# ml-jku/LRAM

Hardware: AMD Instinct MI355X
Metric: env-steps/sec (action-inference) (higher is better)
Workload: dtype f32

## Files before the change

lram_amd/csrc/common.h:

```cpp
#pragma once
#include <hip/hip_runtime.h>
#include <stdint.h>

#include <stdexcept>
#include <string>
#include <type_traits>

namespace lram {

inline bool first_use_on_device(uint64_t& mask) {
  int dev = 0;
  (void)hipGetDevice(&dev);
  const uint64_t bit = 1ull << (dev & 63);
  if (mask & bit) return false;
  mask |= bit;
  return true;
}

struct Error : std::runtime_error {
  using std::runtime_error::runtime_error;
};

#define LRAM_HIP_CHECK(expr)                                                                         \
  do {                                                                                               \
// ... 19 lines not shown
  const float* residual = nullptr;
  int64_t lda = 0, ldw = 0, ldc = 0;
  int m = 0, n = 0, k = 0;
  int nb1 = 1, nb2 = 1;
  int64_t sA1 = 0, sA2 = 0, sW1 = 0, sW2 = 0, sC1 = 0, sC2 = 0, sBias1 = 0, sBias2 = 0;
  const uint16_t* w3 = nullptr;
  int64_t w3_plane = 0;
  const float* gate = nullptr;
  int64_t ldg = 0;
  int act_silu_from = -1;
  const uint16_t* w2 = nullptr;
  int64_t w2_plane = 0, w2_kt = 0;
  const float* w_inv = nullptr;
  const float* a_amax = nullptr;
  int amax_parts = 1;
  const uint16_t* a2 = nullptr;
  int64_t a2_plane = 0, a2_kt = 0;
  const float* a2_inv = nullptr;
  float* splitk_ws = nullptr;
  int64_t splitk_ws_elems = 0;
  const float* a_tab[4] = {nullptr, nullptr, nullptr, nullptr};
  const float* w_tab[4] = {nullptr, nullptr, nullptr, nullptr};
  float* c_tab[4] = {nullptr, nullptr, nullptr, nullptr};
  const uint16_t* w3_tab[4] = {nullptr, nullptr, nullptr, nullptr};
  const float* norm_g = nullptr;
  const float* norm_b = nullptr;
  float norm_eps = 0.f;
  int norm_rms = 0;
  int xcd_gm = 0, xcd_gn = 0;
  int panel_w = 0;
// ... 441 lines not shown
```

lram_amd/csrc/engine.h:

```cpp
#pragma once
#include <algorithm>
#include <array>
#include <cstdlib>
#include <cstring>
#include <map>
#include <memory>
#include <string>
#include <vector>

#include "../../include/lram_hip.h"
#include "common.h"

namespace lram::host {

struct DevBuf {
  float* p = nullptr;
  size_t n = 0;
  void alloc(size_t numel) {
    release();
    if (numel == 0) return;
    LRAM_HIP_CHECK(hipMalloc(reinterpret_cast<void**>(&p), numel * sizeof(float)));
    n = numel;
  }
  void zero(hipStream_t s = nullptr) {
// ... 108 lines not shown
  uint8_t* slot_dev = nullptr;
  int32_t* slot_img_list = nullptr;
  int slot_n_image = 0;
  bool slot_has_discrete = false;
  int lazy_mode = 2;
  bool lazy = false;
  bool lazy_ready = false;
  int lazy_period = 13;
  int gn_fuse = 2;
  bool mamba_dt_fuse = true;
  int slstm_fused_rows = 512;
  int gemm_skinny_rows = 384;
  static constexpr int slstm_gates_rows = 768;
  int gemm_skinny_min = 5;
  static constexpr int gemm_skinny_k = 1024;
  static constexpr int fold_bubbles = 2;
  bool fold_tail = true;
  static constexpr int fold_tail_blocks = 2;
  struct Prefold {
    bool pending = false;
    int blocks = 0;
    int64_t step = 0;
    int period = 0, B = 0;
  } prefold;
  int64_t lazy_step = 0;
  std::vector<int> lazy_bound;
  bool lazy_dirty = false;
  DevBuf LZ_COUNT;
  std::vector<SlotSeg> slot_segs;
  SlotSeg* slot_segs_dev = nullptr;
  SlotChunk* slot_chunks_dev = nullptr;
  int slot_n_chunks = 0, slot_n_rec_chunks = 0;
  int32_t* slot_idx_dev = nullptr;
// ... 168 lines not shown
struct Slice {
  int b0, nb;
  hipStream_t s;
};

struct Pass {
  const uint8_t* images = nullptr;
  int img_c = 0, img_h = 0, img_w = 0;
  bool slots = false;
  int compat_pass = 0, compat_passes = 1;
  bool compat_shared = false;
  const std::vector<hipEvent_t>* lane_wait = nullptr;
  const std::vector<hipEvent_t>* lane_rec = nullptr;
  int n_slices = 1;
  const uint8_t* hold = nullptr;
};

struct ScoreSink {
  float* actions = nullptr;
  int32_t* tokens = nullptr;
  float* logp = nullptr;
  float* logits = nullptr;
  const float* target_actions = nullptr;
  const int32_t* target_tokens = nullptr;
  const uint8_t* valid = nullptr;
  int over = 0;
  double temperature = 1.0;
};

extern thread_local std::string g_last_error;

void alloc_workspace(lram_engine* e, int tokens);
void swap_workspace(lram_engine* e, int lane);
bool twin_ready(lram_engine* e);
int prefill_chunk_steps(lram_engine* e, int L);
bool takes_skinny(const lram_engine* e, const GemmArgs& g);
bool takes_skinny_with_norm(const lram_engine* e, const GemmArgs& g);
bool f16x2_rows(const lram_engine* e, int rows, int n, int k);
bool f16x2_weight(const lram_engine* e, const float* w, int ldw, GemmArgs* g);
bool presplit_for(const lram_engine* e, const float* w, int rows, int n, int k);
void gemm(lram_engine* e, GemmArgs& g, hipStream_t s);
void make_split(lram_engine* e, const float* w, size_t n);
hipEvent_t new_event(const lram_engine* e, bool boundary);
void prof_record(lram_engine* e, hipStream_t s, bool start, bool aux = false);
void prof_tick(lram_engine* e);
hipEvent_t ring_event(lram_engine* e, bool boundary = false);
void stream_after(lram_engine* e, hipStream_t dst, hipStream_t src, bool boundary = false);
std::vector<Slice> make_slices(lram_engine* e, hipStream_t s, hipStream_t* hbm);
void fork_slices(lram_engine* e, const std::vector<Slice>& sl, hipStream_t hbm, hipStream_t s);
void join_slices(lram_engine* e, const std::vector<Slice>& sl, hipStream_t hbm, hipStream_t s);
void save_slot_records(lram_engine* e, const int32_t* host_slots, int n, float* dev_records, hipStream_t s);
void load_slot_records(lram_engine* e, const int32_t* host_slots, int n, const float* dev_records, hipStream_t s);
void lazy_materialize(lram_engine* e, hipStream_t s);
void lazy_finish_prefold(lram_engine* e, hipStream_t s);
void run_xlstm_stack(lram_engine* e, const Pass& pass, int T, const uint8_t* reset, const std::vector<Slice>& sl, hipStream_t hbm);
void run_mamba_stack(lram_engine* e, const Pass& pass, int T, const uint8_t* reset, const std::vector<Slice>& sl);

inline bool has_mlstm_block(const lram_engine* e) {
  if (e->cfg.backbone != LRAM_BACKBONE_XLSTM) return false;
  for (int i = 0; i < e->cfg.n_blocks; ++i)
    if (!e->cfg.block_is_slstm[i]) return true;
  return false;
}
inline double mlstm_block_bytes(const lram_engine* e) {
  if (!has_mlstm_block(e)) return 0.0;
  const double dh = (double)e->cfg.inner / e->cfg.n_heads;
  return (double)e->B * e->cfg.n_heads * dh * dh * 4.0;
}

inline double mlstm_live_bytes(const lram_engine* e) {
  if (!has_mlstm_block(e)) return 0.0;
// ... 36 lines not shown
```

lram_amd/csrc/engine.hip:

```cpp
#include "engine.h"

namespace {

const float* need(lram_engine* e, const std::string& name, size_t numel) {
  auto it = e->weights.find(name);
  if (it == e->weights.end()) throw Error("lram: missing weight '" + name + "'");
  if (it->second.n != numel)
    throw Error("lram: weight '" + name + "' has " + std::to_string(it->second.n) + " elements, expected " +
                std::to_string(numel));
  return it->second.p;
}
const float* optional(lram_engine* e, const std::string& name, size_t numel) {
  auto it = e->weights.find(name);
  if (it == e->weights.end()) return nullptr;
  if (it->second.n != numel)
    throw Error("lram: weight '" + name + "' has " + std::to_string(it->second.n) + " elements, expected " +
                std::to_string(numel));
  return it->second.p;
}

void validate_config(const lram_config& c) {
  LRAM_REQUIRE(c.abi_version == LRAM_ABI_VERSION, "config.abi_version does not match the library");
  LRAM_REQUIRE(c.backbone == LRAM_BACKBONE_XLSTM || c.backbone == LRAM_BACKBONE_MAMBA, "unknown backbone");
  LRAM_REQUIRE(c.d_model > 0 && c.d_model % 4 == 0 && c.d_model <= 2048, "d_model must be a multiple of 4, <= 2048");
// ... 451 lines not shown
  return mlstm_block_bytes(e) >= 128.0 * 1024 * 1024;
}

struct Knob {
  const char* name;
  void (*set)(lram_engine& e, const char* v);
};
const Knob kKnobs[] = {
    {"LRAM_STATE", [](lram_engine& e, const char* v) {
       const std::string m(v);
       e.lazy_mode = m == "lazy" ? 1 : (m == "eager" || m == "materialised" || m == "materialized") ? 0 : 2;
     }},
    {"LRAM_LAZY_PERIOD", [](lram_engine& e, const char* v) { e.lazy_period = std::max(1, std::min(14, std::atoi(v))); }},
    {"LRAM_LAZY_CAP2_ENVS", [](lram_engine& e, const char* v) { e.lazy_cap2_envs = std::max(0, std::atoi(v)); }},
    {"LRAM_FOLD_TAIL", [](lram_engine& e, const char* v) { e.fold_tail = std::atoi(v) != 0; }},
    {"LRAM_GN_FUSE", [](lram_engine& e, const char* v) { e.gn_fuse = std::max(0, std::min(2, std::atoi(v))); }},
    {"LRAM_F16_MIN_ROWS", [](lram_engine& e, const char* v) { e.f16x2_min_rows = std::max(9, std::atoi(v)); }},
    {"LRAM_GEMM_PRESPLIT", [](lram_engine& e, const char* v) { e.gemm_presplit = std::atoi(v) != 0; }},
    {"LRAM_GEMM_NARROW", [](lram_engine& e, const char* v) { e.gemm_narrow_on = std::atoi(v) != 0, e.gemm_narrow_f16 = std::atoi(v) != 2; }},
    {"LRAM_UPZ_8P", [](lram_engine& e, const char* v) { e.upz_beside = std::atoi(v) != 0; }},
    {"LRAM_SLSTM_GATES_ONE", [](lram_engine& e, const char* v) { e.slstm_gates_one = std::atoi(v) != 0; }},
    {"LRAM_GN_AMAX", [](lram_engine& e, const char* v) { e.gn_amax_handover = std::atoi(v) != 0, e.gn_planes = std::atoi(v) >= 2; }},
    {"LRAM_GEMM_SKINNY_ROWS", [](lram_engine& e, const char* v) { e.gemm_skinny_rows = std::max(0, std::atoi(v)); }},
    {"LRAM_GEMM_SKINNY_MIN", [](lram_engine& e, const char* v) { e.gemm_skinny_min = std::max(1, std::atoi(v)); }},
    {"LRAM_SLSTM_FUSED_ROWS", [](lram_engine& e, const char* v) { e.slstm_fused_rows = std::max(0, std::atoi(v)); }},
    {"LRAM_SLSTM_SEQ", [](lram_engine& e, const char* v) { e.slstm_seq = std::atoi(v) != 0, e.slstm_seq_f32 = std::atoi(v) == 2; }},
    {"LRAM_FRONT_MULTI", [](lram_engine& e, const char* v) { e.front_multi = std::atoi(v) != 0; }},
    {"LRAM_FRONT_MIN_ENVS", [](lram_engine& e, const char* v) { e.front_min_envs = std::max(1, std::atoi(v)); }},
    {"LRAM_MAMBA_DT_FUSE", [](lram_engine& e, const char* v) { e.mamba_dt_fuse = std::atoi(v) != 0; }},
    {"LRAM_COMPAT_SHARE", [](lram_engine& e, const char* v) { e.compat_share = std::atoi(v) != 0; }},
// ... 25 lines not shown
      s.conv.alloc((size_t)B * c.conv_k * D);
    } else {
      const size_t DH = e->dh();
      s.s0.alloc((size_t)B * c.n_heads * DH * DH);
      s.n.alloc((size_t)B * c.inner);
      s.m.alloc((size_t)B * c.n_heads);
      s.conv.alloc((size_t)B * c.conv_k * c.inner);
    }
    s.s0.zero();
    s.n.zero();
    s.m.zero();
    s.conv.zero();
  }
  e->B = B;
  e->n_live = B;
  alloc_workspace(e, kMaxTokens);
  e->lazy = lazy_choice(e);
  if (e->lazy) lazy_alloc(e);
  if (e->slot_segs_dev == nullptr) slot_segments_build(e);
  LRAM_HIP_CHECK(hipDeviceSynchronize());
}

}

extern "C" {

const char* lram_last_error(void) { return g_last_error.c_str(); }

int32_t lram_abi_version(void) { return LRAM_ABI_VERSION; }

// ... 251 lines not shown
```

lram_amd/csrc/engine_gemm.hip:

```cpp
#include "engine.h"

namespace lram::host {

bool takes_skinny(const lram_engine* e, const GemmArgs& g) {
  const bool shape = g.k <= e->gemm_skinny_k && (g.m <= e->gemm_skinny_rows / 2 || (int64_t)g.n * g.k <= 600000);
  return g.m >= e->gemm_skinny_min && g.m <= e->gemm_skinny_rows && shape && gemm_skinny_supported(g);
}
bool takes_skinny_with_norm(const lram_engine* e, const GemmArgs& g) {
  return takes_skinny(e, g) && gemm_skinny_norm_supported(g);
}

}

namespace {

bool narrow_takes(const lram_engine* e, const GemmArgs& g) {
  if (!e->gemm_narrow_on || g.m < e->gemm_narrow_min_rows || g.a2 != nullptr || (int)g.ldw != g.k) return false;
  return e->narrow.count(g.w) != 0 && gemm_narrow_supported(g);
}

}

namespace lram::host {

// ... 11 lines not shown
  if (g != nullptr) {
    g->w2 = it->second.planes + row0 * 32;
    g->w2_plane = (int64_t)split_f16x2_plane_elems(it->second.rows, it->second.k), g->w2_kt = (int64_t)it->second.rows * 32;
    g->w_inv = it->second.inv + row0;
  }
  return true;
}

bool presplit_for(const lram_engine* e, const float* w, int rows, int n, int k) {
  if (!e->gemm_presplit || (k & 31) != 0 || e->XN2.p == nullptr || !f16x2_rows(e, rows, n, k)) return false;
  GemmArgs probe;
  if ((int64_t)e->XN2.n * 4 >= (1ll << 31) || !f16x2_weight(e, w, k, &probe)) return false;
  return 4 * probe.w2_plane < (1ll << 31);
}

void gemm(lram_engine* e, GemmArgs& g, hipStream_t s) {
  if (e->SK.p != nullptr) {
    g.splitk_ws = e->SK.p + (size_t)stream_slot(e, s) * lram_engine::kSplitKSlotElems;
    g.splitk_ws_elems = (int64_t)lram_engine::kSplitKSlotElems;
  }
  if (g.a2 != nullptr) {
    LRAM_REQUIRE(f16x2_weight(e, g.w, (int)g.ldw, &g) && gemm_f16x2p_supported(g),
                 "gemm: pre-split A operand for a projection the pre-split kernel does not serve");
    launch_gemm_f16x2p(g, s);
    count_gemm(e, 0, g);
    return;
  }
  if (narrow_takes(e, g)) {
    if (e->use_f16x2 && e->gemm_narrow_f16 && g.a_amax != nullptr && f16x2_weight(e, g.w, (int)g.ldw, &g) && gemm_narrow16_supported(g)) {
      launch_gemm_narrow16(g, s);
      count_gemm(e, 0, g);
      return;
    }
    g.w2 = nullptr, g.w_inv = nullptr, g.w2_kt = 0;
    launch_gemm_narrow(g, e->narrow.find(g.w)->second.p, s);
    count_gemm(e, 2, g);
    return;
  }
  if (f16x2_rows(e, g.m, g.n, g.k) && g.nb1 * g.nb2 == 1 && e->ASCALE.p != nullptr && (size_t)g.m <= e->ascale_rows) {
    if (f16x2_weight(e, g.w, (int)g.ldw, &g) && gemm_f16x2_supported(g)) {
      if (g.a_amax == nullptr) {
        float* sc = e->ASCALE.p + (size_t)stream_slot(e, s) * e->ascale_rows;
        launch_row_amax(g.a, g.lda, g.gate, g.ldg, g.m, g.k, sc, s);
        g.a_amax = sc, g.amax_parts = 1;
      }
      launch_gemm_f16x2(g, s);
      count_gemm(e, 0, g);
      return;
    }
    g.w2 = nullptr, g.w_inv = nullptr, g.w2_kt = 0;
  }
  if (takes_skinny(e, g)) {
    launch_gemm_skinny(g, s);
    count_gemm(e, 3, g);
    return;
  }
  if (e->use_bf16x3 && !gemm_small_m(g)) {
    auto it = e->split.upper_bound(g.w);
    if (it != e->split.begin() && (--it, g.w < it->first + it->second.n)) {
      g.w3 = it->second.p + (g.w - it->first);
      g.w3_plane = (int64_t)it->second.n;
      if (gemm_bf16x3_supported(g)) {
        launch_gemm_bf16x3(g, s);
        count_gemm(e, 1, g);
        return;
      }
// ... 169 lines not shown
```

lram_amd/csrc/engine_step.hip:

```cpp
#include "engine.h"

namespace {

void run_stack(lram_engine* e, Pass pass, int T, const uint8_t* reset, const std::vector<Slice>& sl, hipStream_t hbm) {
  pass.n_slices = (int)sl.size();
  if (e->cfg.backbone == LRAM_BACKBONE_MAMBA)
    run_mamba_stack(e, pass, T, reset, sl);
  else
    run_xlstm_stack(e, pass, T, reset, sl, hbm);
}

struct ImageFrameFloats {
  size_t p, x;
};
ImageFrameFloats image_frame_floats(int H, int W) {
  const size_t hp = (H - 1) / 2 + 1, wp = (W - 1) / 2 + 1;
  const size_t x = 32 * hp * wp;
  return {std::max((size_t)16 * H * W, x), x};
}

void image_buffers(lram_engine* e, int C, int H, int W, const char* who) {
  const std::string wh(who);
  LRAM_REQUIRE(e->img_lin_w != nullptr, wh + ": no embed_image.* weights were uploaded");
  LRAM_REQUIRE(C == e->img_channels, wh + ": channel count " + std::to_string(C) +
// ... 178 lines not shown
  const lram_config& c = e->cfg;
  const int D = c.d_model, T = c.tokens_per_step;
  const int64_t nlog = (int64_t)c.act_dim * c.n_vocab;
  const int pred = T * (last_steps - 1) + c.pred_token;
  const int col_begin = pass.compat_pass;
  const int col_end = (pass.compat_shared && col_begin + 1 < pass.compat_passes) ? col_begin + 1 : c.act_dim;
  const int col0 = pass.compat_shared ? col_begin : 0;
  e->last_head = discrete;
  const HeadGeom geom = head_geom(c);
  for (const Slice& x : sl) {
    const size_t r0 = (size_t)x.b0 * Tc, b0 = x.b0;
    GemmArgs gh;
    gh.a = e->HID.p + (r0 + pred) * D, gh.lda = (int64_t)Tc * D, gh.w = e->w_head + (size_t)col0 * c.n_vocab * D, gh.ldw = D;
    gh.c = e->LOGITS.p + b0 * nlog + (size_t)col0 * c.n_vocab, gh.ldc = nlog, gh.bias = e->b_head + (size_t)col0 * c.n_vocab;
    gh.m = x.nb, gh.n = (col_end - col0) * c.n_vocab, gh.k = D;
    gemm(e, gh, x.s);
    if (sink != nullptr) {
      ScoreArgs a = score_args(e, *sink, discrete);
      a.logits = e->LOGITS.p + b0 * nlog, a.ld = nlog, a.row0 = (int64_t)b0, a.rows = x.nb;
      a.inner = 1, a.outer = L, a.off = L - 1, a.start = ctx_start;
      launch_action_score(a, x.s);
      continue;
    }
    const float* logits = e->LOGITS.p + b0 * nlog;
    float* act = actions + b0 * c.act_dim;
    int32_t* tok = tokens ? tokens + b0 * c.act_dim : nullptr;
    const HeadSlots slots = head_slots(e, discrete, b0);
    if (e->sampling) {
      SampleArgs sp = e->sample;
      sp.slot0 += b0, sp.draw = e->sample_draw;
// ... 132 lines not shown
bool compat_shares(const lram_engine* e, int discrete) {
  const int passes = discrete ? 1 : std::max(1, std::min(e->compat_repeat, e->cfg.act_dim));
  return passes > 1 && e->cfg.backbone == LRAM_BACKBONE_MAMBA && e->compat_share && e->cfg.n_blocks >= 2;
}
void compat_prepare(lram_engine* e, int discrete) {
  if (e->B <= 0 || !compat_shares(e, discrete)) return;
  const size_t bt = (size_t)e->B * e->cfg.tokens_per_step;
  if (e->X0.n < bt * e->cfg.d_model) e->X0.alloc(bt * e->cfg.d_model);
  if (e->U0.n < bt * 2 * e->cfg.d_inner) e->U0.alloc(bt * 2 * e->cfg.d_inner);
}

void step_launches(lram_engine* e, Pass pass, const Inputs& in, const uint8_t* reset, int discrete, float* actions,
                   int32_t* tokens, hipStream_t s) {
  pass.compat_passes = discrete ? 1 : std::max(1, std::min(e->compat_repeat, e->cfg.act_dim));
  pass.compat_shared = compat_shares(e, discrete);
  if (pass.compat_shared) {
    const size_t bt = (size_t)e->n_live * e->cfg.tokens_per_step;
    LRAM_REQUIRE(e->X0.n >= bt * e->cfg.d_model && e->U0.n >= bt * 2 * e->cfg.d_inner,
                 "shared repeated forwards: workspace not prepared");
  }
  for (pass.compat_pass = 0; pass.compat_pass < pass.compat_passes; ++pass.compat_pass)
    timesteps_launches(e, pass, in, pass.compat_pass == 0 ? reset : nullptr, discrete, actions, tokens, s);
  sample_draw_advance(e, s);
}

void require_all_live(const lram_engine* e, const char* who) {
  LRAM_REQUIRE(e->n_live == e->B, std::string(who) + ": " + std::to_string(e->B - e->n_live) + " of " + std::to_string(e->B) +
                                      " env slots are parked (lram_set_live): stored contexts and encoder calls need every slot "
                                      "live -- call lram_set_live(batch) first");
}
// ... 188 lines not shown
        if (!e->capture_stream) LRAM_HIP_CHECK(hipStreamCreateWithFlags(&e->capture_stream, hipStreamNonBlocking));
        hipStream_t cs = e->capture_stream;
        LRAM_HIP_CHECK(hipStreamBeginCapture(cs, hipStreamCaptureModeThreadLocal));
        try {
          step_launches(e, Pass{}, in, dev_reset_mask, discrete, dev_actions, dev_tokens, cs);
        } catch (...) {
          hipGraph_t g = nullptr;
          (void)hipStreamEndCapture(cs, &g);
          if (g) (void)hipGraphDestroy(g);
          throw;
        }
        LRAM_HIP_CHECK(hipStreamEndCapture(cs, &e->graph));
        LRAM_HIP_CHECK(hipGraphInstantiate(&e->graph_exec, e->graph, nullptr, nullptr, 0));
        e->graph_key = key;
        e->graph_valid = true;
      }
      LRAM_HIP_CHECK(hipGraphLaunch(e->graph_exec, s));
    } else {
      step_launches(e, Pass{}, in, dev_reset_mask, discrete, dev_actions, dev_tokens, s);
    }
  });
}

int32_t lram_step_images(lram_engine* e, const uint8_t* dev_images, int32_t channels, int32_t height, int32_t width,
                         const float* dev_rtg, const float* dev_reward, const uint8_t* dev_reset_mask, int32_t discrete,
                         float* dev_actions, int32_t* dev_tokens, void* stream) {
  return guarded([&] {
    step_entry(e, "lram_step_images");
    LRAM_REQUIRE(dev_images && dev_rtg && dev_reward && dev_actions && channels > 0 && height > 0 && width > 0,
                 "lram_step_images: bad argument");
    LRAM_REQUIRE(e->img_lin_w != nullptr, "lram_step_images: no embed_image.* weights were uploaded");
    check_head_mode(e, discrete, "lram_step_images");
// ... 218 lines not shown
    LRAM_HIP_CHECK(hipMemcpyAsync(dev_hidden_out, e->HID.p, bytes, hipMemcpyDeviceToDevice, s));
  });
}

int32_t lram_get_taps(lram_engine* e, float* dev_tokens_embed, float* dev_hidden, float* dev_logits, void* stream) {
  return guarded([&] {
    LRAM_REQUIRE(e && e->B > 0, "lram_get_taps: state not allocated");
    hipStream_t s = static_cast<hipStream_t>(stream);
    const size_t btd = sizeof(float) * (size_t)e->n_live * e->cfg.tokens_per_step * e->cfg.d_model;
    if (dev_tokens_embed) {
      LRAM_REQUIRE(e->B <= kTokenTapMaxBatch,
                   "lram_get_taps: the embed_ln token tap is kept for batches of up to 1024 env slots only (it costs a "
                   "copy of the token buffer per step); pass NULL for it");
      LRAM_HIP_CHECK(hipMemcpyAsync(dev_tokens_embed, e->TOK.p, btd, hipMemcpyDeviceToDevice, s));
    }
    if (dev_hidden) LRAM_HIP_CHECK(hipMemcpyAsync(dev_hidden, e->HID.p, btd, hipMemcpyDeviceToDevice, s));
    if (dev_logits)
      LRAM_HIP_CHECK(hipMemcpyAsync(dev_logits, e->LOGITS.p, sizeof(float) * (e->LOGITS.n / e->B) * e->n_live, hipMemcpyDeviceToDevice, s));
  });
}

int32_t lram_sample_tokens(const float* dev_logits, int64_t rows, int32_t n, int64_t ld, double temperature, int32_t top_k,
                           double top_p, const double* dev_uniform, int32_t* dev_tokens, void* stream) {
  return guarded([&] {
    LRAM_REQUIRE(dev_logits && dev_uniform && dev_tokens, "lram_sample_tokens: null device pointer");
    LRAM_REQUIRE(temperature > 0.0 && temperature < (double)INFINITY, "lram_sample_tokens: temperature must be finite and > 0");
    LRAM_REQUIRE(top_p >= 0.0 && top_p <= 1.0, "lram_sample_tokens: top_p must be in [0, 1]");
    LRAM_REQUIRE(top_k >= 0 && top_k <= n, "lram_sample_tokens: top_k must be in 0 .. n");
    LRAM_REQUIRE(ld == 0 || ld >= n, "lram_sample_tokens: ld must be 0 (one shared row) or >= n");
    launch_sample_tokens(dev_logits, rows, n, ld, temperature, top_k, top_p, dev_uniform, dev_tokens,
                         static_cast<hipStream_t>(stream));
// ... 24 lines not shown
```

lram_amd/csrc/engine_xlstm.hip:

```cpp
#include "engine.h"

namespace {

MlstmLazyArgs lazy_args(lram_engine* e, int i, int T, const uint8_t* reset, int b0, int nb, int step_off = 0) {
  const lram_config& c = e->cfg;
  const size_t NH = c.n_heads, DH = e->dh(), B = e->B;
  const int64_t step = e->lazy_step + step_off;
  const int in = (int)(step & 1), out = 1 - in;
  BlockState& st = e->st[i];
  MlstmLazyArgs a{};
  a.C = st.s0.p + (size_t)b0 * NH * DH * DH;
  a.wk = st.wk.p + (size_t)b0 * NH * kLazyWindow * DH;
  a.wv = st.wv.p + (size_t)b0 * NH * kLazyWindow * DH;
  a.coef_in = st.coef.p + (in * B + b0) * NH * kLazyWindow;
  a.coef_out = st.coef.p + (out * B + b0) * NH * kLazyWindow;
  a.g_in = st.gsc.p + (in * B + b0) * NH;
  a.g_out = st.gsc.p + (out * B + b0) * NH;
  a.count_in = reinterpret_cast<const int32_t*>(e->LZ_COUNT.p) + in * B + b0;
  a.count_out = reinterpret_cast<int32_t*>(e->LZ_COUNT.p) + out * B + b0;
  a.pw = st.pw.p ? st.pw.p + (size_t)b0 * NH * T * kLazyWT : nullptr;
  a.reset = reset ? reset + b0 : nullptr;
  a.B = nb, a.T = T, a.NH = (int)NH, a.DH = (int)DH;
  a.phase = (int)((step + b0) % e->lazy_period), a.period = e->lazy_period, a.force = 0;
  return a;
// ... 174 lines not shown
  ca.reset = reset ? reset + b0 : nullptr, ca.B = sl.nb, ca.T = T, ca.NH = NH, ca.DH = DH;
  ca.hold = pass.hold ? pass.hold + b0 : nullptr;
  const long wgs = (long)sl.nb * NH * ((DH % 256 == 0) ? DH / 256 : (DH % 128 == 0) ? DH / 128 : DH / 64);
  ca.min_lds_bytes = wgs >= 1024 ? 84 * 1024 : 0;
  ca.unroll = e->cell_unroll;
  if (T > kMaxTokens) {
    ca.amat = e->AMAT.p + b0 * NH * kChunkMaxTokens * kChunkMaxTokens;
    ca.vec = e->VEC.p + b0 * NH * 3 * kChunkMaxTokens;
    ca.chunk_exact_fp32 = e->chunk_exact_fp32 ? 1 : 0;
  }
  prof_record(e, s, true);
  launch_mlstm_cell(ca, s);
  prof_record(e, s, false);
}

void mlstm_back(lram_engine* e, const Pass& pass, int i, int T, const Slice& sl) {
  const lram_config& c = e->cfg;
  const int D = c.d_model, inner = c.inner, NH = c.n_heads, DH = e->dh(), rows = sl.nb * T;
  const size_t r0 = (size_t)sl.b0 * T;
  const BlockWeights& w = e->bw[i];
  float* X = e->X.p + r0 * D;
  if (gn_fused(e, T)) {
    GemmArgs dn;
    dn.a = e->H.p + r0 * e->icols, dn.lda = inner, dn.w = w.proj_down, dn.ldw = inner, dn.c = X, dn.ldc = D, dn.residual = X;
    dn.m = rows, dn.n = D, dn.k = inner;
    dn.gate = e->U.p + r0 * e->ucols + inner, dn.ldg = 2 * inner;
    gemm(e, dn, sl.s);
    return;
  }
  GroupNormArgs ga;
  ga.h = e->H.p + r0 * e->icols, ga.gamma = w.on_g, ga.beta = w.on_b, ga.skip = w.skip, ga.xa = e->XA.p + r0 * e->icols;
  ga.u = e->U.p + r0 * e->ucols, ga.out = e->G.p + r0 * e->icols, ga.rows = rows, ga.NH = NH, ga.DH = DH, ga.mode = 0;
  ga.eps = c.ln_eps;
  const bool hand_over = e->gn_amax_handover && e->AMX_H.p != nullptr && f16x2_rows(e, rows, D, inner);
  GemmArgs dn;
  dn.a = e->G.p + r0 * e->icols, dn.lda = inner, dn.w = w.proj_down, dn.ldw = inner, dn.c = X, dn.ldc = D, dn.residual = X;
  dn.m = rows, dn.n = D, dn.k = inner;
  const int64_t bt = (int64_t)(e->G.n / e->icols);
  GemmArgs probe;
  const bool planes = hand_over && e->gn_planes && pass.n_slices == 1 && e->gemm_presplit && NH <= 8 && (inner & 31) == 0 && bt * inner * 4 < (1ll << 31) &&
                      f16x2_weight(e, w.proj_down, inner, &probe) && 4 * probe.w2_plane < (1ll << 31);
  if (planes) {
    ga.out = nullptr;
    ga.h2 = reinterpret_cast<uint16_t*>(e->G.p) + r0 * 32, ga.h2_plane = bt * inner, ga.h2_kt = bt * 32, ga.h2_inv = e->AMX_H.p + r0;
    dn.a = nullptr, dn.a2 = ga.h2, dn.a2_plane = ga.h2_plane, dn.a2_kt = ga.h2_kt, dn.a2_inv = ga.h2_inv;
  } else {
    ga.amax = hand_over ? e->AMX_H.p + r0 * NH : nullptr;
    if (hand_over) dn.a_amax = ga.amax, dn.amax_parts = NH;
  }
  launch_group_norm(ga, sl.s);
  gemm(e, dn, sl.s);
}

bool slstm_gates_one_bf16x3(const lram_engine* e, GemmArgs& g4, const BlockWeights& w, const float* XC, const float* XN, float* gates,
                            int Hs) {
  if (!e->use_bf16x3 || !e->slstm_gates_one) return false;
  int64_t plane = -1;
  for (int g = 0; g < 4; ++g) {
    auto it = e->split.find(w.gate_w[g]);
    if (it == e->split.end() || (plane >= 0 && (int64_t)it->second.n != plane)) return false;
    plane = (int64_t)it->second.n;
    g4.a_tab[g] = (g < 2) ? XC : XN, g4.w_tab[g] = w.gate_w[g], g4.c_tab[g] = gates + (int64_t)g * Hs;
    g4.w3_tab[g] = it->second.p;
  }
  g4.w3 = g4.w3_tab[0], g4.w3_plane = plane;
// ... 107 lines not shown
  launch_gelu_gate(Ubuf, Gbuf, rows, F, s);
  GemmArgs dn;
  dn.a = Gbuf, dn.lda = F, dn.w = w.ffn_down, dn.ldw = F, dn.c = X, dn.ldc = D, dn.residual = X;
  dn.m = rows, dn.n = D, dn.k = F;
  gemm(e, dn, s);
}

}

namespace lram::host {

void run_xlstm_stack(lram_engine* e, const Pass& pass, int T, const uint8_t* reset, const std::vector<Slice>& sl, hipStream_t hbm) {
  const lram_config& c = e->cfg;
  const int D = c.d_model;
  const bool lazy = lazy_active(e, T);
  LRAM_REQUIRE(!(lazy && pass.hold != nullptr), "xLSTM stack: the lazy kernels have no hold rule (stored contexts run materialised)");
  int n_prefolded = 0;
  if (e->prefold.pending) {
    const lram_engine::Prefold& pf = e->prefold;
    if (lazy && sl.size() > 1 && pass.lane_rec == nullptr && pf.step == e->lazy_step && pf.period == e->lazy_period && pf.B == e->B &&
        lazy_bound_compact(e, e->lazy_step, T)) {
      n_prefolded = pf.blocks;
      e->prefold = lram_engine::Prefold{};
    } else {
      lazy_finish_prefold(e, hbm);
      for (const Slice& x : sl) stream_after(e, x.s, hbm);
    }
  }
  bool lazy_compact = false;
  if (lazy) {
// ... 22 lines not shown
    stream_after(e, fold_stream, sl[0].s);
  }
  std::vector<char> folded(c.n_blocks, 0);
  auto launch_folds = [&](int i) {
    fold_block(e, i, T, reset, lazy_compact, 0, fold_stream);
    folded[i] = 1;
  };
  auto next_mlstm = [&](int i) {
    for (int k = i + 1; k < c.n_blocks; ++k)
      if (!c.block_is_slstm[k]) return k;
    return -1;
  };
  for (int i = next_mlstm(-1), k = 0; i >= 0 && k < n_prefolded; i = next_mlstm(i), ++k) folded[i] = 1;
  if (bubbles) {
    int k = 0;
    const int ahead = pass.images != nullptr ? e->fold_bubbles_images : lram_engine::fold_bubbles;
    for (int i = next_mlstm(-1); i >= 0 && k < ahead; i = next_mlstm(i))
      if (!folded[i]) launch_folds(i), ++k;
  }
  int last_mlstm = -1;
  for (int i = next_mlstm(-1); i >= 0; i = next_mlstm(i)) last_mlstm = i;
  const bool tail = bubbles && e->fold_tail && lazy_compact && pass.lane_rec == nullptr && lazy_bound_compact(e, e->lazy_step + 1, T);
  if (side_folds)
    for (int i = next_mlstm(-1); i >= 0; i = next_mlstm(i)) {
      launch_folds(i);
      fold_done[i] = ring_event(e);
      LRAM_HIP_CHECK(hipEventRecord(fold_done[i], fold_stream));
    }
  for (int i = 0; i < c.n_blocks; ++i) {
    if (i > 0 && pass.lane_rec) LRAM_HIP_CHECK(hipEventRecord((*pass.lane_rec)[i - 1], sl[0].s));
    if (pass.lane_wait) LRAM_HIP_CHECK(hipStreamWaitEvent(sl[0].s, (*pass.lane_wait)[i], 0));
// ... 37 lines not shown
        prof_record(e, hbm, true);
        launch_mlstm_lazy_cell(la, hbm);
        prof_record(e, hbm, false);
        mlstm_up_z(e, i, T, x);
        stream_after(e, x.s, hbm);
        continue;
      }
      stream_after(e, hbm, x.s);
      mlstm_cell(e, pass, i, T, reset, x, hbm);
      mlstm_up_z(e, i, T, x);
      stream_after(e, x.s, hbm);
    }
    if (tail && i == last_mlstm) {
      e->prefold.step = e->lazy_step + 1, e->prefold.period = e->lazy_period, e->prefold.B = e->B, e->prefold.blocks = 0;
      e->prefold.pending = true;
      for (int k = next_mlstm(-1); k >= 0 && e->prefold.blocks < lram_engine::fold_tail_blocks; k = next_mlstm(k)) {
        fold_block(e, k, T, nullptr, true, 1, hbm);
        ++e->prefold.blocks;
      }
    }
    for (const Slice& x : sl) mlstm_back(e, pass, i, T, x);
  }
  if (pass.lane_rec) LRAM_HIP_CHECK(hipEventRecord((*pass.lane_rec)[c.n_blocks - 1], sl[0].s));
  if (lazy) {
    ++e->lazy_step;
    e->lazy_dirty = true;
  }
  for (const Slice& x : sl) {
    const size_t r0 = (size_t)x.b0 * T;
    launch_row_norm(e->X.p + r0 * D, D, e->HID.p + r0 * D, D, e->post_g, e->post_b, x.nb * T, D, c.ln_eps,
                    c.norm_is_rms, x.s);
  }
}

}
```

lram_amd/csrc/gemm_f16x2.hip:

```cpp
#include <algorithm>
#include <cstdlib>

#include "gemm_f16x2_tile.h"

namespace lram {

namespace {
constexpr int BN = 128, BK = 32;
constexpr int kPitchPadded = 40;

template <bool HAS_BIAS, bool HAS_RES, int BM, bool GATE, bool DB = false>
__global__ __launch_bounds__(256, DB ? 2 : 3) void gemm_f16x2_kernel(GemmArgs g) {
  constexpr int WM = BM / 2;
  constexpr int TI = WM / 32;
  constexpr int PITCH = DB ? 32 : kPitchPadded;
  constexpr int PLANE = BN * PITCH;
  constexpr int APLANE = BM * PITCH;
  constexpr int STAGE = 2 * APLANE + 2 * PLANE;
  __shared__ __attribute__((aligned(16))) _Float16 lds[(DB ? 2 : 1) * STAGE];
  float* srow = reinterpret_cast<float*>(lds);
  __shared__ float sinv[DB ? 1 : BM + BN];
  _Float16* As = lds;
  _Float16* Bs = lds + 2 * APLANE;

  const int tid = threadIdx.x, lane = tid & 63, wave = tid >> 6;
  const int wm = wave >> 1, wn = wave & 1;
  const float* A = g.a;
  const _Float16* W2 = reinterpret_cast<const _Float16*>(g.w2);

  const int tiles_n = (g.n + BN - 1) / BN;
  const int tiles_m = (g.m + BM - 1) / BM;
  int tm_idx, tn_idx;
  gemm_tile_of(g, blockIdx.x, tiles_m, tiles_n, tm_idx, tn_idx);
  const int m0 = tm_idx * BM, n0 = tn_idx * BN;

  if (tid < BM) {
    const int gm = m0 + tid;
    float mx = 0.f;
    if (gm < g.m) {
      const float* ap = g.a_amax + (int64_t)gm * g.amax_parts;
      for (int q = 0; q < g.amax_parts; ++q) mx = fmaxf(mx, ap[q]);
    }
    srow[tid] = gm < g.m ? pow2_scale(mx) : 0.f;
    if (!DB) sinv[tid] = gm < g.m ? 1.f / pow2_scale(mx) : 0.f;
  } else if (!DB && tid < BM + BN) {
    sinv[tid] = g.w_inv[min(n0 + tid - BM, g.n - 1)];
  }
  __syncthreads();
  const int lr = tid >> 3;
  const int lc = (tid & 7) << 2;
  constexpr int NA = BM / 32;
  constexpr int NSET = DB ? 2 : 1;
  float4 ra[NSET][NA];
  float4 rz[NSET][GATE ? NA : 1];
  (void)rz;
// ... 206 lines not shown

void launch_row_amax(const float* a, int64_t lda, const float* gate, int64_t ldg, int rows, int k, float* amax,
                     hipStream_t stream) {
  LRAM_REQUIRE((k & 3) == 0 && (lda & 3) == 0 && (gate == nullptr || (ldg & 3) == 0), "row amax: K, lda must be multiples of 4");
  hipLaunchKernelGGL(row_amax_kernel, dim3((unsigned)((rows + 3) / 4)), dim3(256), 0, stream, a, lda, gate, ldg, rows, k, amax);
  LRAM_HIP_CHECK(hipGetLastError());
}

void launch_split_f16x2(const float* w, int rows, int k, uint16_t* planes, float* inv, hipStream_t stream) {
  hipLaunchKernelGGL(split_f16x2_kernel, dim3((unsigned)((rows + 3) / 4)), dim3(256), 0, stream, w, rows, k,
                     reinterpret_cast<_Float16*>(planes), (int64_t)split_f16x2_plane_elems(rows, k), inv);
  LRAM_HIP_CHECK(hipGetLastError());
}

template <int BM, bool GATE>
static void launch_bm(const GemmArgs& g, dim3 grid, hipStream_t stream) {
  const long wgs = (long)grid.x * grid.y * grid.z;
  launch_bias_res(g, [&](auto b, auto r) {
    constexpr bool hb = decltype(b)::value, hr = decltype(r)::value;
    if (wgs <= 256 && !GATE)
      hipLaunchKernelGGL((gemm_f16x2_kernel<hb, hr, BM, false, true>), grid, dim3(256), 0, stream, g);
    else
      hipLaunchKernelGGL((gemm_f16x2_kernel<hb, hr, BM, GATE, false>), grid, dim3(256), 0, stream, g);
  });
}

void launch_gemm_f16x2(const GemmArgs& g_in, hipStream_t stream) {
  GemmArgs g = g_in;
  g.mfma_prio = 1;
  LRAM_REQUIRE(g.m > 0 && g.n > 0 && g.k > 0, "gemm: empty problem");
  LRAM_REQUIRE(gemm_f16x2_supported(g) && g.a_amax != nullptr, "gemm f16x2: unsupported operand layout");
  int S = 1;
  if (g.act_silu_from >= 0 || g.gate != nullptr)
    g.split_k = 1, g.k_tiles_per_split = 0;
  else
    S = gemm_choose_split_k(g);
  const int tiles_n = (g.n + BN - 1) / BN;
  const int tiles128 = ((g.m + 127) / 128) * tiles_n;
  const int force_bm = gemm_knobs().tile;
  const bool forced = force_bm == 64 || force_bm == 128;
  const bool small = gemm_f16x2p_tile(g, S) == 64 || (!forced && g.m > 64 && S == 1 && tiles128 < 768 && tiles_n <= 6);
  const int tiles = small ? ((g.m + 63) / 64) * tiles_n : tiles128;
  dim3 grid(tiles, 1, S);
  gemm_choose_xcd_split(g, small ? 64 : 128, BN, 4);
  if (g.gate != nullptr) {
    if (small) launch_bm<64, true>(g, grid, stream); else launch_bm<128, true>(g, grid, stream);
  } else {
    if (small) launch_bm<64, false>(g, grid, stream); else launch_bm<128, false>(g, grid, stream);
  }
  LRAM_HIP_CHECK(hipGetLastError());
  if (S > 1) launch_splitk_reduce(g, stream);
}

}
```

Baseline: 464,200.

## Compute last-block down projection and post-norm only for the prediction token rows

In the xLSTM stack, the final block's down projection and the post-norm now run only on the rows of the token that feeds the action head, using strided row subsets through the f16x2 GEMM. The remaining token rows are computed lazily in complete_hidden, and only when the caller asks for hidden states. Tile and split-k choices still follow the full row count so the GEMM configuration stays the same. The cost is extra bookkeeping, including a copy of the tail state kept for graph replay, and a risk of stale hidden rows if some path reads HID without calling complete_hidden. Fold-bubble counts also become runtime-tunable.

```diff
diff --git a/lram_amd/csrc/common.h b/lram_amd/csrc/common.h
--- a/lram_amd/csrc/common.h
+++ b/lram_amd/csrc/common.h
@@ -57,6 +57,8 @@
   const float* w_inv = nullptr;
   const float* a_amax = nullptr;
   int amax_parts = 1;
+  int64_t amax_ld = 0;
+  int m_hint = 0;
   const uint16_t* a2 = nullptr;
   int64_t a2_plane = 0, a2_kt = 0;
   const float* a2_inv = nullptr;
diff --git a/lram_amd/csrc/engine.h b/lram_amd/csrc/engine.h
--- a/lram_amd/csrc/engine.h
+++ b/lram_amd/csrc/engine.h
@@ -146,9 +146,20 @@
   static constexpr int slstm_gates_rows = 768;
   int gemm_skinny_min = 5;
   static constexpr int gemm_skinny_k = 1024;
-  static constexpr int fold_bubbles = 2;
+  int fold_bubbles = 2;
   bool fold_tail = true;
-  static constexpr int fold_tail_blocks = 2;
+  int fold_tail_blocks = 2;
+  bool pred_rows = true;
+  struct HidTail {
+    bool pending = false;
+    int T = 0, pred = 0;
+    struct Part {
+      int b0 = 0, nb = 0;
+      bool has_dn = false;
+      GemmArgs dn;
+    };
+    std::vector<Part> parts;
+  } hid_tail, graph_hid_tail;
   struct Prefold {
     bool pending = false;
     int blocks = 0;
@@ -347,6 +358,7 @@
   const std::vector<hipEvent_t>* lane_rec = nullptr;
   int n_slices = 1;
   const uint8_t* hold = nullptr;
+  bool pred_rows = false;
 };
 
 struct ScoreSink {
@@ -370,6 +382,7 @@
 bool takes_skinny(const lram_engine* e, const GemmArgs& g);
 bool takes_skinny_with_norm(const lram_engine* e, const GemmArgs& g);
 bool f16x2_rows(const lram_engine* e, int rows, int n, int k);
+bool takes_f16x2(const lram_engine* e, const GemmArgs& g);
 bool f16x2_weight(const lram_engine* e, const float* w, int ldw, GemmArgs* g);
 bool presplit_for(const lram_engine* e, const float* w, int rows, int n, int k);
 void gemm(lram_engine* e, GemmArgs& g, hipStream_t s);
@@ -388,6 +401,7 @@
 void lazy_finish_prefold(lram_engine* e, hipStream_t s);
 void run_xlstm_stack(lram_engine* e, const Pass& pass, int T, const uint8_t* reset, const std::vector<Slice>& sl, hipStream_t hbm);
 void run_mamba_stack(lram_engine* e, const Pass& pass, int T, const uint8_t* reset, const std::vector<Slice>& sl);
+void complete_hidden(lram_engine* e, hipStream_t s);
 
 inline bool has_mlstm_block(const lram_engine* e) {
   if (e->cfg.backbone != LRAM_BACKBONE_XLSTM) return false;
diff --git a/lram_amd/csrc/engine.hip b/lram_amd/csrc/engine.hip
--- a/lram_amd/csrc/engine.hip
+++ b/lram_amd/csrc/engine.hip
@@ -489,6 +489,9 @@
     {"LRAM_LAZY_PERIOD", [](lram_engine& e, const char* v) { e.lazy_period = std::max(1, std::min(14, std::atoi(v))); }},
     {"LRAM_LAZY_CAP2_ENVS", [](lram_engine& e, const char* v) { e.lazy_cap2_envs = std::max(0, std::atoi(v)); }},
     {"LRAM_FOLD_TAIL", [](lram_engine& e, const char* v) { e.fold_tail = std::atoi(v) != 0; }},
+    {"LRAM_FOLD_BUBBLES", [](lram_engine& e, const char* v) { e.fold_bubbles = std::max(0, std::min(64, std::atoi(v))); }},
+    {"LRAM_FOLD_TAIL_BLOCKS", [](lram_engine& e, const char* v) { e.fold_tail_blocks = std::max(0, std::min(64, std::atoi(v))); }},
+    {"LRAM_PRED_ROWS", [](lram_engine& e, const char* v) { e.pred_rows = std::atoi(v) != 0; }},
     {"LRAM_GN_FUSE", [](lram_engine& e, const char* v) { e.gn_fuse = std::max(0, std::min(2, std::atoi(v))); }},
     {"LRAM_F16_MIN_ROWS", [](lram_engine& e, const char* v) { e.f16x2_min_rows = std::max(9, std::atoi(v)); }},
     {"LRAM_GEMM_PRESPLIT", [](lram_engine& e, const char* v) { e.gemm_presplit = std::atoi(v) != 0; }},
@@ -544,6 +547,7 @@
   }
   e->B = B;
   e->n_live = B;
+  e->hid_tail = lram_engine::HidTail{}, e->graph_hid_tail = lram_engine::HidTail{};
   alloc_workspace(e, kMaxTokens);
   e->lazy = lazy_choice(e);
   if (e->lazy) lazy_alloc(e);
diff --git a/lram_amd/csrc/engine_gemm.hip b/lram_amd/csrc/engine_gemm.hip
--- a/lram_amd/csrc/engine_gemm.hip
+++ b/lram_amd/csrc/engine_gemm.hip
@@ -49,11 +49,23 @@
   return 4 * probe.w2_plane < (1ll << 31);
 }
 
+static bool f16x2_shape(const lram_engine* e, const GemmArgs& g) {
+  return f16x2_rows(e, std::max(g.m, g.m_hint), g.n, g.k) && g.nb1 * g.nb2 == 1 && e->ASCALE.p != nullptr &&
+         (size_t)std::max(g.m, g.m_hint) <= e->ascale_rows;
+}
+bool takes_f16x2(const lram_engine* e, const GemmArgs& g) {
+  if (g.a2 != nullptr || narrow_takes(e, g) || !f16x2_shape(e, g)) return false;
+  GemmArgs probe = g;
+  return f16x2_weight(e, g.w, (int)g.ldw, &probe) && gemm_f16x2_supported(probe);
+}
+
 void gemm(lram_engine* e, GemmArgs& g, hipStream_t s) {
   if (e->SK.p != nullptr) {
     g.splitk_ws = e->SK.p + (size_t)stream_slot(e, s) * lram_engine::kSplitKSlotElems;
     g.splitk_ws_elems = (int64_t)lram_engine::kSplitKSlotElems;
   }
+  LRAM_REQUIRE((g.m_hint == 0 && g.amax_ld == 0) || takes_f16x2(e, g),
+               "gemm: a row subset of a projection (m_hint / amax_ld) needs the f16x2 kernel");
   if (g.a2 != nullptr) {
     LRAM_REQUIRE(f16x2_weight(e, g.w, (int)g.ldw, &g) && gemm_f16x2p_supported(g),
                  "gemm: pre-split A operand for a projection the pre-split kernel does not serve");
@@ -72,7 +84,7 @@
     count_gemm(e, 2, g);
     return;
   }
-  if (f16x2_rows(e, g.m, g.n, g.k) && g.nb1 * g.nb2 == 1 && e->ASCALE.p != nullptr && (size_t)g.m <= e->ascale_rows) {
+  if (f16x2_shape(e, g)) {
     if (f16x2_weight(e, g.w, (int)g.ldw, &g) && gemm_f16x2_supported(g)) {
       if (g.a_amax == nullptr) {
         float* sc = e->ASCALE.p + (size_t)stream_slot(e, s) * e->ascale_rows;
@@ -85,6 +97,7 @@
     }
     g.w2 = nullptr, g.w_inv = nullptr, g.w2_kt = 0;
   }
+  LRAM_REQUIRE(g.m_hint == 0 && g.amax_ld == 0, "gemm: a row subset of a projection (m_hint / amax_ld) needs the f16x2 kernel");
   if (takes_skinny(e, g)) {
     launch_gemm_skinny(g, s);
     count_gemm(e, 3, g);
diff --git a/lram_amd/csrc/engine_step.hip b/lram_amd/csrc/engine_step.hip
--- a/lram_amd/csrc/engine_step.hip
+++ b/lram_amd/csrc/engine_step.hip
@@ -216,6 +216,7 @@
     gh.a = e->HID.p + (r0 + pred) * D, gh.lda = (int64_t)Tc * D, gh.w = e->w_head + (size_t)col0 * c.n_vocab * D, gh.ldw = D;
     gh.c = e->LOGITS.p + b0 * nlog + (size_t)col0 * c.n_vocab, gh.ldc = nlog, gh.bias = e->b_head + (size_t)col0 * c.n_vocab;
     gh.m = x.nb, gh.n = (col_end - col0) * c.n_vocab, gh.k = D;
+    if (pass.pred_rows && e->hid_tail.pending && last_steps == 1 && e->use_f16x2 && takes_f16x2(e, gh)) gh.a_amax = e->AMX_XN.p + r0;
     gemm(e, gh, x.s);
     if (sink != nullptr) {
       ScoreArgs a = score_args(e, *sink, discrete);
@@ -378,6 +379,7 @@
                    int32_t* tokens, hipStream_t s) {
   pass.compat_passes = discrete ? 1 : std::max(1, std::min(e->compat_repeat, e->cfg.act_dim));
   pass.compat_shared = compat_shares(e, discrete);
+  pass.pred_rows = true;
   if (pass.compat_shared) {
     const size_t bt = (size_t)e->n_live * e->cfg.tokens_per_step;
     LRAM_REQUIRE(e->X0.n >= bt * e->cfg.d_model && e->U0.n >= bt * 2 * e->cfg.d_inner,
@@ -596,8 +598,10 @@
         LRAM_HIP_CHECK(hipGraphInstantiate(&e->graph_exec, e->graph, nullptr, nullptr, 0));
         e->graph_key = key;
         e->graph_valid = true;
+        e->graph_hid_tail = e->hid_tail;
       }
       LRAM_HIP_CHECK(hipGraphLaunch(e->graph_exec, s));
+      e->hid_tail = e->graph_hid_tail;
     } else {
       step_launches(e, Pass{}, in, dev_reset_mask, discrete, dev_actions, dev_tokens, s);
     }
@@ -846,7 +850,10 @@
                    "copy of the token buffer per step); pass NULL for it");
       LRAM_HIP_CHECK(hipMemcpyAsync(dev_tokens_embed, e->TOK.p, btd, hipMemcpyDeviceToDevice, s));
     }
-    if (dev_hidden) LRAM_HIP_CHECK(hipMemcpyAsync(dev_hidden, e->HID.p, btd, hipMemcpyDeviceToDevice, s));
+    if (dev_hidden) {
+      complete_hidden(e, s);
+      LRAM_HIP_CHECK(hipMemcpyAsync(dev_hidden, e->HID.p, btd, hipMemcpyDeviceToDevice, s));
+    }
     if (dev_logits)
       LRAM_HIP_CHECK(hipMemcpyAsync(dev_logits, e->LOGITS.p, sizeof(float) * (e->LOGITS.n / e->B) * e->n_live, hipMemcpyDeviceToDevice, s));
   });
diff --git a/lram_amd/csrc/engine_xlstm.hip b/lram_amd/csrc/engine_xlstm.hip
--- a/lram_amd/csrc/engine_xlstm.hip
+++ b/lram_amd/csrc/engine_xlstm.hip
@@ -212,7 +212,17 @@
   prof_record(e, s, false);
 }
 
-void mlstm_back(lram_engine* e, const Pass& pass, int i, int T, const Slice& sl) {
+bool down_rows_of_token(const lram_engine* e, GemmArgs& dn, int T, int tok) {
+  if (T <= 1 || dn.m % T != 0 || !takes_f16x2(e, dn)) return false;
+  dn.m_hint = dn.m, dn.m /= T;
+  dn.a += tok * dn.lda, dn.lda *= T;
+  dn.c += tok * dn.ldc, dn.residual += tok * dn.ldc, dn.ldc *= T;
+  if (dn.gate != nullptr) dn.gate += tok * dn.ldg, dn.ldg *= T;
+  if (dn.a_amax != nullptr) dn.a_amax += (int64_t)tok * dn.amax_parts, dn.amax_ld = (int64_t)T * dn.amax_parts;
+  return true;
+}
+
+void mlstm_back(lram_engine* e, const Pass& pass, int i, int T, const Slice& sl, lram_engine::HidTail::Part* tail = nullptr) {
   const lram_config& c = e->cfg;
   const int D = c.d_model, inner = c.inner, NH = c.n_heads, DH = e->dh(), rows = sl.nb * T;
   const size_t r0 = (size_t)sl.b0 * T;
@@ -223,6 +233,7 @@
     dn.a = e->H.p + r0 * e->icols, dn.lda = inner, dn.w = w.proj_down, dn.ldw = inner, dn.c = X, dn.ldc = D, dn.residual = X;
     dn.m = rows, dn.n = D, dn.k = inner;
     dn.gate = e->U.p + r0 * e->ucols + inner, dn.ldg = 2 * inner;
+    if (tail != nullptr && down_rows_of_token(e, dn, T, c.pred_token)) tail->has_dn = true, tail->dn = dn;
     gemm(e, dn, sl.s);
     return;
   }
@@ -247,6 +258,7 @@
     if (hand_over) dn.a_amax = ga.amax, dn.amax_parts = NH;
   }
   launch_group_norm(ga, sl.s);
+  if (tail != nullptr && !planes && hand_over && down_rows_of_token(e, dn, T, c.pred_token)) tail->has_dn = true, tail->dn = dn;
   gemm(e, dn, sl.s);
 }
 
@@ -384,6 +396,13 @@
   const lram_config& c = e->cfg;
   const int D = c.d_model;
   const bool lazy = lazy_active(e, T);
+  const bool pred_rows = pass.pred_rows && e->pred_rows && T == c.tokens_per_step && T > 1 && pass.lane_rec == nullptr && pass.hold == nullptr;
+  e->hid_tail = lram_engine::HidTail{};
+  if (pred_rows) {
+    e->hid_tail.T = T, e->hid_tail.pred = c.pred_token;
+    e->hid_tail.parts.resize(sl.size());
+    for (size_t k = 0; k < sl.size(); ++k) e->hid_tail.parts[k].b0 = sl[k].b0, e->hid_tail.parts[k].nb = sl[k].nb;
+  }
   LRAM_REQUIRE(!(lazy && pass.hold != nullptr), "xLSTM stack: the lazy kernels have no hold rule (stored contexts run materialised)");
   int n_prefolded = 0;
   if (e->prefold.pending) {
@@ -436,7 +455,7 @@
   for (int i = next_mlstm(-1), k = 0; i >= 0 && k < n_prefolded; i = next_mlstm(i), ++k) folded[i] = 1;
   if (bubbles) {
     int k = 0;
-    const int ahead = pass.images != nullptr ? e->fold_bubbles_images : lram_engine::fold_bubbles;
+    const int ahead = pass.images != nullptr ? e->fold_bubbles_images : e->fold_bubbles;
     for (int i = next_mlstm(-1); i >= 0 && k < ahead; i = next_mlstm(i))
       if (!folded[i]) launch_folds(i), ++k;
   }
@@ -504,12 +523,12 @@
     if (tail && i == last_mlstm) {
       e->prefold.step = e->lazy_step + 1, e->prefold.period = e->lazy_period, e->prefold.B = e->B, e->prefold.blocks = 0;
       e->prefold.pending = true;
-      for (int k = next_mlstm(-1); k >= 0 && e->prefold.blocks < lram_engine::fold_tail_blocks; k = next_mlstm(k)) {
+      for (int k = next_mlstm(-1); k >= 0 && e->prefold.blocks < e->fold_tail_blocks; k = next_mlstm(k)) {
         fold_block(e, k, T, nullptr, true, 1, hbm);
         ++e->prefold.blocks;
       }
     }
-    for (const Slice& x : sl) mlstm_back(e, pass, i, T, x);
+    for (size_t k = 0; k < sl.size(); ++k) mlstm_back(e, pass, i, T, sl[k], (pred_rows && i == c.n_blocks - 1) ? &e->hid_tail.parts[k] : nullptr);
   }
   if (pass.lane_rec) LRAM_HIP_CHECK(hipEventRecord((*pass.lane_rec)[c.n_blocks - 1], sl[0].s));
   if (lazy) {
@@ -518,9 +537,40 @@
   }
   for (const Slice& x : sl) {
     const size_t r0 = (size_t)x.b0 * T;
+    if (pred_rows) {
+      const size_t at = (r0 + c.pred_token) * D;
+      launch_row_norm(e->X.p + at, (int64_t)T * D, e->HID.p + at, (int64_t)T * D, e->post_g, e->post_b, x.nb, D, c.ln_eps,
+                      c.norm_is_rms, x.s, nullptr, e->use_f16x2 ? e->AMX_XN.p + r0 : nullptr);
+      continue;
+    }
     launch_row_norm(e->X.p + r0 * D, D, e->HID.p + r0 * D, D, e->post_g, e->post_b, x.nb * T, D, c.ln_eps,
                     c.norm_is_rms, x.s);
   }
-}
-
-}
+  e->hid_tail.pending = pred_rows;
+}
+
+void complete_hidden(lram_engine* e, hipStream_t s) {
+  if (!e->hid_tail.pending) return;
+  const lram_engine::HidTail ht = e->hid_tail;
+  e->hid_tail.pending = false;
+  LRAM_HIP_CHECK(hipSetDevice(e->device));
+  const lram_config& c = e->cfg;
+  const int D = c.d_model, T = ht.T;
+  for (const lram_engine::HidTail::Part& p : ht.parts)
+    for (int tok = 0; tok < T; ++tok) {
+      if (tok == ht.pred) continue;
+      const int64_t d = tok - ht.pred;
+      if (p.has_dn) {
+        GemmArgs dn = p.dn;
+        dn.a += d * (dn.lda / T), dn.c += d * (dn.ldc / T), dn.residual += d * (dn.ldc / T);
+        if (dn.gate != nullptr) dn.gate += d * (dn.ldg / T);
+        if (dn.amax_ld != 0) dn.a_amax += d * (dn.amax_ld / T);
+        gemm(e, dn, s);
+      }
+      const size_t at = ((size_t)p.b0 * T + tok) * D;
+      launch_row_norm(e->X.p + at, (int64_t)T * D, e->HID.p + at, (int64_t)T * D, e->post_g, e->post_b, p.nb, D, c.ln_eps,
+                      c.norm_is_rms, s);
+    }
+}
+
+}
diff --git a/lram_amd/csrc/gemm_f16x2.hip b/lram_amd/csrc/gemm_f16x2.hip
--- a/lram_amd/csrc/gemm_f16x2.hip
+++ b/lram_amd/csrc/gemm_f16x2.hip
@@ -38,7 +38,7 @@
     const int gm = m0 + tid;
     float mx = 0.f;
     if (gm < g.m) {
-      const float* ap = g.a_amax + (int64_t)gm * g.amax_parts;
+      const float* ap = g.a_amax + (int64_t)gm * (g.amax_ld != 0 ? g.amax_ld : (int64_t)g.amax_parts);
       for (int q = 0; q < g.amax_parts; ++q) mx = fmaxf(mx, ap[q]);
     }
     srow[tid] = gm < g.m ? pow2_scale(mx) : 0.f;
@@ -275,8 +275,7 @@
 }
 
 template <int BM, bool GATE>
-static void launch_bm(const GemmArgs& g, dim3 grid, hipStream_t stream) {
-  const long wgs = (long)grid.x * grid.y * grid.z;
+static void launch_bm(const GemmArgs& g, dim3 grid, long wgs, hipStream_t stream) {
   launch_bias_res(g, [&](auto b, auto r) {
     constexpr bool hb = decltype(b)::value, hr = decltype(r)::value;
     if (wgs <= 256 && !GATE)
@@ -291,23 +290,27 @@
   g.mfma_prio = 1;
   LRAM_REQUIRE(g.m > 0 && g.n > 0 && g.k > 0, "gemm: empty problem");
   LRAM_REQUIRE(gemm_f16x2_supported(g) && g.a_amax != nullptr, "gemm f16x2: unsupported operand layout");
+  GemmArgs d = g;
+  if (g.m_hint > g.m) d.m = g.m_hint;
   int S = 1;
   if (g.act_silu_from >= 0 || g.gate != nullptr)
     g.split_k = 1, g.k_tiles_per_split = 0;
   else
-    S = gemm_choose_split_k(g);
+    S = gemm_choose_split_k(d), g.split_k = d.split_k, g.k_tiles_per_split = d.k_tiles_per_split;
   const int tiles_n = (g.n + BN - 1) / BN;
-  const int tiles128 = ((g.m + 127) / 128) * tiles_n;
+  const int tiles128 = ((d.m + 127) / 128) * tiles_n;
   const int force_bm = gemm_knobs().tile;
   const bool forced = force_bm == 64 || force_bm == 128;
-  const bool small = gemm_f16x2p_tile(g, S) == 64 || (!forced && g.m > 64 && S == 1 && tiles128 < 768 && tiles_n <= 6);
-  const int tiles = small ? ((g.m + 63) / 64) * tiles_n : tiles128;
+  const bool small = gemm_f16x2p_tile(d, S) == 64 || (!forced && d.m > 64 && S == 1 && tiles128 < 768 && tiles_n <= 6);
+  const int bm = small ? 64 : 128;
+  const int tiles = ((g.m + bm - 1) / bm) * tiles_n;
+  const long wgs = (long)((d.m + bm - 1) / bm) * tiles_n * S;
   dim3 grid(tiles, 1, S);
-  gemm_choose_xcd_split(g, small ? 64 : 128, BN, 4);
+  gemm_choose_xcd_split(g, bm, BN, 4);
   if (g.gate != nullptr) {
-    if (small) launch_bm<64, true>(g, grid, stream); else launch_bm<128, true>(g, grid, stream);
+    if (small) launch_bm<64, true>(g, grid, wgs, stream); else launch_bm<128, true>(g, grid, wgs, stream);
   } else {
-    if (small) launch_bm<64, false>(g, grid, stream); else launch_bm<128, false>(g, grid, stream);
+    if (small) launch_bm<64, false>(g, grid, wgs, stream); else launch_bm<128, false>(g, grid, wgs, stream);
   }
   LRAM_HIP_CHECK(hipGetLastError());
   if (S > 1) launch_splitk_reduce(g, stream);
```

Result: slower. 458,700 (-1.2%).
